# Amos-Chen98/neo-planner

Measured on NVIDIA B200. Metric: optimized trajectories/sec to convergence, higher is better.
Workload: dtype f64

## Files before the change

### neo_planner_b200/csrc/lbfgsb_tile.cuh

```cuda
#pragma once
#include "minco_tile.cuh"
#include "x87_nrm2.h"

namespace neo {

#ifdef NEO_OPT_TICKS
#define OT_BEGIN long long ot_last = clock64()
#define OT(i) do { const long long ot_now = clock64(); if (T.tl == 0) { atomicAdd((unsigned long long *)&g_opt_ticks[i], (unsigned long long)(ot_now - ot_last)); atomicAdd((unsigned long long *)&g_opt_ticks[32 + (i)], 1ull); } ot_last = clock64(); } while (0)
#else
#define OT_BEGIN do { } while (0)
#define OT(i) do { } while (0)
#endif

__device__ __forceinline__ double xmul(double a, double b) { return __dmul_rn(a, b); }
__device__ __forceinline__ double xadd(double a, double b) { return __dadd_rn(a, b); }
__device__ __forceinline__ double xsub(double a, double b) { return __dsub_rn(a, b); }
__device__ __noinline__ double xdiv(double a, double b) { return __ddiv_rn(a, b); }
__device__ __noinline__ double xsqrt(double a) { return __dsqrt_rn(a); }
__device__ __noinline__ double nrm2_x87(int n, const double *v) { return x87_nrm2(n, v); }
__device__ __forceinline__ double xrcp(double a) { return __drcp_rn(a); }
__device__ __forceinline__ double xfma(double a, double b, double c) { return __fma_rn(a, b, c); }
__device__ __forceinline__ double xdiv_r(double a, double b, double rb)
{
    const double q = __dmul_rn(a, rb);
// ... 377 lines not shown
#pragma unroll 1
    for (int i = m2 - 1; i >= 0; i--) {
        const double *ui = wn + wn_col(i);
        if (T.tl == 0) wv[i] = xdiv_r(wv[i], ui[i], rd[i]);
        T.sync();
        const double t = -wv[i];
#pragma unroll 1
        for (int k = T.tl; k < i; k += TL) wv[k] = xfma(t, ui[k], wv[k]);
        T.sync();
    }
    OT(10);
    if (T.tl < n) {
#pragma unroll 1
        for (int jy = 0; jy < col; jy++) {
            const int sj = lb_slot(L, jy);
            d = xadd(xadd(d, xdiv_r(xmul(m.wy[sj * n + T.tl], wv[jy]), theta, rtheta)), xmul(m.ws[sj * n + T.tl], wv[col + jy]));
        }
        d = xmul(d, rtheta);
    }
    T.sync();
    OT(11);
    return d;
}

template <int TL>
__device__ __forceinline__ void ls_load(const Tile<TL> &T, const double *p, Dcsrch &S)
{
    S.finit = p[0]; S.ginit = p[1]; S.gtest = p[2]; S.width = p[3]; S.width1 = p[4]; S.stx = p[5]; S.fx = p[6]; S.gx = p[7];
    S.sty = p[8]; S.fy = p[9]; S.gy = p[10]; S.stmin = p[11]; S.stmax = p[12];
    const int flags = (int)p[13];
    S.brackt = (flags & 1) != 0; S.stage = flags >> 1;
}
template <int TL>
__device__ __forceinline__ void ls_store(const Tile<TL> &T, double *p, const Dcsrch &S)
{
    T.sync();
    if (T.tl == 0) {
        p[0] = S.finit; p[1] = S.ginit; p[2] = S.gtest; p[3] = S.width; p[4] = S.width1; p[5] = S.stx; p[6] = S.fx; p[7] = S.gx;
        p[8] = S.sty; p[9] = S.fy; p[10] = S.gy; p[11] = S.stmin; p[12] = S.stmax;
        p[13] = (double)((S.brackt ? 1 : 0) | (S.stage << 1));
    }
    T.sync();
}

constexpr int ST_CANCELLED = 7;
constexpr int ST_RUNNING = -1;

struct OptState {
    double x, g, d, t, r, z, xlast;
    double f, stp, gd;
    LbMem L;
    int nit, nfev, ifun, status;
    bool first;
};

__device__ __forceinline__ void opt_begin(OptState &o, double x0l)
{
    o.x = x0l; o.g = 0.0; o.d = 0.0; o.t = 0.0; o.r = 0.0; o.z = 0.0; o.xlast = 0.0;
    o.f = 0.0; o.stp = 0.0; o.gd = 0.0;
    o.L.col = 0; o.L.head = 0; o.L.iupdat = 0; o.L.theta = 1.0;
    o.nit = 0; o.nfev = 0; o.ifun = 0; o.status = ST_RUNNING; o.first = true;
}

template <int TL>
__device__ __forceinline__ bool opt_same_point(const Tile<TL> &T, const OptState &o, int n)
{
    return !o.first && T.all(T.tl >= n || o.x == o.xlast);
}

template <int TL, int NC>
__device__ __forceinline__ double opt_gd(const Tile<TL> &T, const TileMem &m, int n, double g, double d)
{
    T.sync();
    if (T.tl < n) { m.gv[T.tl] = g; m.dv[T.tl] = d; }
    T.sync();
    return blas_ddot_n<NC>(m.gv, m.dv, n);
}

template <int TL, int NC>
__device__ __forceinline__ void opt_advance(const Tile<TL> &T, const TileMem &m, int n, OptState &o,
                                            const unsigned *cancel_word, unsigned cancel_mask)
{
    const bool mine = T.tl < n;
    const double pgtol = 1e-4, ftol = 1e-4, epsmch = 2.220446049250313e-16;
    const double tol = (ftol / epsmch) * epsmch;
    const int maxls = 20, maxiter = 15000, maxfun = 15000;
    bool new_dir;
    OT_BEGIN;
    if (o.first) {
        o.first = false;
        if (T.dmax(mine ? fabs(o.g) : 0.0) <= pgtol) { o.status = 1; return; }
        new_dir = true;
    } else {
        o.gd = opt_gd<TL, NC>(T, m, n, o.g, o.d);
        Dcsrch ls;
        ls_load(T, m.ls, ls);
        const int ls_task = dcsrch_step(ls, o.stp, o.f, o.gd);
        if (ls_task == 0) ls_store(T, m.ls, ls);
        OT(0);
        if (ls_task == 0) new_dir = false;
        else {
            o.nit++;
            if (cancel_mask) {
                unsigned w = 0;
                if (T.tl == 0) w = *reinterpret_cast<const volatile unsigned *>(cancel_word);
                if (T.shfl(w, 0) & cancel_mask) { o.status = ST_CANCELLED; return; }
            }
            if (T.dmax(mine ? fabs(o.g) : 0.0) <= pgtol) { o.status = 1; return; }
            const double fold = m.ls[14], gdold = m.ls[15];
            if (xsub(fold, o.f) <= xmul(tol, max3(fabs(fold), fabs(o.f), 1.0))) { o.status = 0; return; }
            if (o.nit >= maxiter || o.nfev > maxfun) { o.status = 3; return; }
            const double y = xsub(o.g, o.r);
            T.sync();
            if (mine) m.dv[T.tl] = y;
            T.sync();
            OT(12);
            const double nr = nrm2_x87(n, m.dv);
            const double rr = xmul(nr, nr);
            OT(1);
            double dr, ddum, s;
            if (o.stp == 1.0) { dr = xsub(o.gd, gdold); ddum = -gdold; s = o.d; }
            else { dr = xmul(xsub(o.gd, gdold), o.stp); s = xmul(o.d, o.stp); ddum = xmul(-gdold, o.stp); }
            if (!(dr <= xmul(epsmch, ddum))) lb_update<TL, NC>(T, m, n, o.L, s, y, rr, dr);
            new_dir = true;
        }
    }
    for (;;) {
        if (new_dir) {
            OT(15);
            if (o.L.col > 0 && !lb_factor(T, m, o.L)) { o.L.col = 0; o.L.head = 0; o.L.iupdat = 0; o.L.theta = 1.0; }
            if (o.L.col == 0) o.z = xsub(o.x, o.g);
            else o.z = xadd(o.x, lb_step<TL, NC>(T, m, n, o.L, o.g));
            o.d = mine ? xsub(o.z, o.x) : 0.0;
            T.sync();
            if (mine) m.dv[T.tl] = o.d;
            T.sync();
            OT(13);
            const double dnorm = nrm2_x87(n, m.dv);
            OT(1);
            o.stp = (o.nit == 0) ? fmin(xdiv(1.0, dnorm), LS_STPMAX) : 1.0;
            o.t = o.x; o.r = o.g;
            o.gd = opt_gd<TL, NC>(T, m, n, o.g, o.d);
            T.sync();
            if (T.tl == 0) { m.ls[14] = o.f; m.ls[15] = o.gd; }
            o.ifun = 0;
            if (o.gd >= 0.0) o.ifun = maxls + 1;
            else { Dcsrch ls; dcsrch_start(ls, o.stp, o.f, o.gd); ls_store(T, m.ls, ls); }
            OT(14);
        }
        o.ifun++;
        if (o.ifun - 1 < maxls) break;
        T.sync();
        o.x = o.t; o.g = o.r; o.f = m.ls[14];
        if (o.L.col == 0) { o.status = 2; return; }
        o.L.col = 0; o.L.head = 0; o.L.iupdat = 0; o.L.theta = 1.0;
        new_dir = true;
    }
    o.x = (o.stp == 1.0) ? o.z : xadd(xmul(o.stp, o.d), o.t);
}

}
```

### neo_planner_b200/csrc/neoopt.cu

```cuda
#include <cuda_runtime.h>
#include <math.h>
#include <stdio.h>
#include <stdlib.h>
#include <string.h>

#include <algorithm>
#include <atomic>
#include <chrono>
#include <condition_variable>
#include <functional>
#include <mutex>
#include <thread>
#include <string>
#include <vector>

#include "../../include/neoopt.h"
#include "astar_warp.cuh"
#include "lbfgsb_tile.cuh"
#include "map_kernels.cuh"
#include "minco_tile.cuh"

using namespace neo;

constexpr int WARPS_PER_CTA = 4;
#ifndef NEO_GROUPED_MIN_PROBLEMS
#define NEO_GROUPED_MIN_PROBLEMS 2048
#endif
#ifndef NEO_TILE_MIN_PROBLEMS
#define NEO_TILE_MIN_PROBLEMS 12288
#endif
#ifndef NEO_HOST_THREADS
#define NEO_HOST_THREADS 8
#endif

struct OptArgs {
    int B, M, max_attempts;
    const double *x0;
    const int32_t *x0_status;
    const double *head, *tail;
    const int32_t *map_ids;
    const double *retry_q;
    const double *retry_tau;
    int retry_status;
    const MapView *maps;
    unsigned int *counter;
    double *t_x;
    double *t_costs;
    int32_t *t_info;
    long long *t_work;
    unsigned int *p_state;
    double *x, *ts, *coeffs, *costs;
    int32_t *status, *ok, *attempt, *nit, *runs, *nfev;
    long long *work;
    int trace_cap;
    int bus_q;
    double *tr_x, *tr_f, *tr_g, *tr_costs;
    int32_t *tr_status, *tr_len;
};

__device__ __forceinline__ bool resolved(unsigned st, int A)
{
    const unsigned done = st & 0xffu, okm = (st >> 8) & 0xffu;
    if (okm) { const unsigned lower = (1u << (__ffs(okm) - 1)) - 1u; return (done & lower) == lower; }
    return done == (1u << A) - 1u;
}

#ifdef NEO_ROUND_TRACE
__device__ long long g_round_trace[12 * 2048 * 4];
#endif
template <int MODE, int MC, int TL, int MINB, int WPC = WARPS_PER_CTA>
__global__ void __launch_bounds__(WPC * 32, MINB) k_optimize(const DevParams P, const OptArgs a)
{
    extern __shared__ double smem[];
    const int lane = threadIdx.x & 31, warp = threadIdx.x >> 5;
    const Tile<TL> T(lane);
    constexpr int TPW = 32 / TL;
    const int M = MC > 0 ? MC : a.M, n = 3 * M - 2, nq = 2 * (M - 1), N = 6 * M, A = a.max_attempts;
    constexpr bool ONE_BLOCK = MODE == SAMPLE_BY_PIECE_STAGED;
    const TileMem m = carve(smem + (size_t)(warp * TPW + lane / TL) * tile_mem_doubles(M, TL, ONE_BLOCK), M, TL, ONE_BLOCK);
    const unsigned total = (unsigned)A * (unsigned)a.B;
    const bool mine = T.tl < n;
    OptState o;
    opt_begin(o, 0.0);
    bool running = false, retired = false;
    unsigned tid = 0, lower_ok = 0;
    int at = 0;
    size_t b = 0;
    int map_id = 0;
    unsigned long long t_start = 0;
    __shared__ unsigned s_arrivals;
    constexpr unsigned BUS_DRAIN = 0x80000000u;
    bool drained = false;
    if constexpr (WPC > WARPS_PER_CTA) {
        if (threadIdx.x == 0) s_arrivals = 0;
        __syncthreads();
    }
#ifdef NEO_ROUND_TRACE
    int rt_round = 0;
#endif
    for (;;) {
#ifdef NEO_ROUND_TRACE
        if (blockIdx.x == 0 && lane == 0 && rt_round < 2048) g_round_trace[(warp * 2048 + rt_round) * 4 + 0] = clock64();
#endif
        if constexpr (WPC > WARPS_PER_CTA) {
            __syncwarp();
            if (!drained) {
                unsigned k = 0;
                if (lane == 0) k = atomicAdd(&s_arrivals, 1u);
                k = __shfl_sync(FULL, k, 0);
                if (k & BUS_DRAIN) drained = true;
                else asm volatile("bar.sync %0, %1;" ::"r"(1 + (int)((k / (unsigned)a.bus_q) & 7u)), "r"(a.bus_q * 32) : "memory");
            }
        }
#ifdef NEO_ROUND_TRACE
        if (blockIdx.x == 0 && lane == 0 && rt_round < 2048) g_round_trace[(warp * 2048 + rt_round) * 4 + 1] = clock64();
        const int rt_now = rt_round++;
#endif
// ... 100 lines not shown
            }
            if (accepted) bits |= 1u << (8 + at);
            __threadfence();
        }
        T.sync();
        unsigned old = 0;
        if (T.tl == 0) old = atomicOr(a.p_state + b, bits);
        old = T.shfl(old, 0);
        const unsigned now = old | bits;
        if (!resolved(now, A) || resolved(old, A)) continue;

        __threadfence();
        const unsigned okm = (now >> 8) & 0xffu;
        const int last = okm ? __ffs(okm) - 1 : A - 1;
        int nit = 0, runs = 0, nfev = 0, src = -1, status = 0;
        long long ns = 0, nv = 0, nc = 0, nanos = 0;
        for (int k = 0; k <= last; k++) {
            const size_t t = (size_t)k * a.B + b;
            const int st = __ldcg(a.t_info + t * 4 + 0);
            status = st;
            nfev += __ldcg(a.t_info + t * 4 + 2);
            ns += __ldcg(a.t_work + t * 4 + 0); nv += __ldcg(a.t_work + t * 4 + 1); nc += __ldcg(a.t_work + t * 4 + 2);
            nanos += __ldcg(a.t_work + t * 4 + 3);
            if (__ldcg(a.t_info + t * 4 + 3)) { runs++; nit += __ldcg(a.t_info + t * 4 + 1); src = k; }
        }
        if (src >= 0) {
            const size_t t = (size_t)src * a.B + b;
            const double xf = mine ? __ldcg(a.t_x + t * n + T.tl) : 0.0;
            begin_problem(T, m, M, a.head + b * 6, a.tail + b * 6);
            double e_unused;
            times_from_tau(T, P, m, M, xf, e_unused);
            load_nodes(T, m, M, xf);
            solve_nodes(T, m, M);
            hermite_coeffs(T, m, M);
            if (mine) a.x[b * n + T.tl] = xf;
            if (T.tl < M) a.ts[b * M + T.tl] = m.ts[T.tl];
            for (int i = T.tl; i < 2 * N; i += TL) a.coeffs[b * 2 * N + i] = m.c[i];
            if (T.tl < 4) a.costs[b * 4 + T.tl] = __ldcg(a.t_costs + t * 4 + T.tl);
        } else {
            if (mine) a.x[b * n + T.tl] = 0.0;
            if (T.tl < M) a.ts[b * M + T.tl] = 0.0;
            for (int i = T.tl; i < 2 * N; i += TL) a.coeffs[b * 2 * N + i] = 0.0;
            if (T.tl < 4) a.costs[b * 4 + T.tl] = 0.0;
        }
        if (T.tl == 0) {
            a.status[b] = status; a.ok[b] = okm ? 1 : 0; a.attempt[b] = last; a.nit[b] = nit; a.runs[b] = runs;
            a.nfev[b] = nfev;
            if (a.work) { a.work[b * 4] = ns; a.work[b * 4 + 1] = nv; a.work[b * 4 + 2] = nc; a.work[b * 4 + 3] = nanos; }
        }
        T.sync();
    }
}

struct EvalArgs {
    int B, M;
    const double *x, *head, *tail;
    const int32_t *map_ids;
    const MapView *maps;
    double *costs, *grad, *coeffs, *ts;
    int32_t *status;
};

template <int MODE, int MC, int TL>
__global__ void __launch_bounds__(WARPS_PER_CTA * 32, 3) k_eval(const DevParams P, const EvalArgs a)
{
    extern __shared__ double smem[];
    const int lane = threadIdx.x & 31, warp = threadIdx.x >> 5;
    const Tile<TL> T(lane);
    constexpr int TPW = 32 / TL, TPC = WARPS_PER_CTA * TPW;
    const int M = MC > 0 ? MC : a.M, n = 3 * M - 2, N = 6 * M;
    const int tile = warp * TPW + lane / TL;
    constexpr bool ONE_BLOCK = MODE == SAMPLE_BY_PIECE_STAGED;
    const TileMem m = carve(smem + (size_t)tile * eval_mem_doubles(M, TL, ONE_BLOCK), M, TL, ONE_BLOCK, true);
    for (size_t b = (size_t)blockIdx.x * TPC + tile; b < (size_t)a.B; b += (size_t)gridDim.x * TPC) {
        begin_problem(T, m, M, a.head + b * 6, a.tail + b * 6);
        const MapView map = a.maps[a.map_ids ? a.map_ids[b] : 0];
        const double xl = T.tl < n ? a.x[b * n + T.tl] : 0.0;
        EvalOut ev;
        eval_fg<MODE, TL, true>(T, P, map, m, M, xl, true, ev);
        if (T.tl < n) a.grad[b * n + T.tl] = ev.status ? 0.0 : ev.g;
        if (T.tl < 4) a.costs[b * 4 + T.tl] = ev.costs[T.tl];
        if (T.tl == 0) a.status[b] = ev.status;
        if (a.coeffs) for (int i = T.tl; i < 2 * N; i += TL) a.coeffs[b * 2 * N + i] = ev.status == NEO_ST_OVERFLOW ? 0.0 : m.c[i];
        if (a.ts && T.tl < M) a.ts[b * M + T.tl] = m.ts[T.tl];
        T.sync();
    }
}

__global__ void __launch_bounds__(WARPS_PER_CTA * 32) k_coeffs(int B, int M, const double *q, const double *ts,
                                                               const double *head, const double *tail, double *coeffs)
{
    extern __shared__ double smem[];
    const int lane = threadIdx.x & 31, warp = threadIdx.x >> 5;
    const Tile<32> T(lane);
    const int nq = 2 * (M - 1), N = 6 * M;
    const TileMem m = carve(smem + (size_t)warp * tile_mem_doubles(M), M);
    for (size_t b = (size_t)blockIdx.x * WARPS_PER_CTA + warp; b < (size_t)B; b += (size_t)gridDim.x * WARPS_PER_CTA) {
        begin_problem(T, m, M, head + b * 6, tail + b * 6);
        if (lane < M) {
            const double Tt = ts[b * M + lane];
            m.ts[lane] = Tt;
            const double a = 1.0 / Tt, a2 = a * a;
            double *it = m.iT + 5 * lane;
            it[0] = a; it[1] = a2; it[2] = a2 * a; it[3] = a2 * a2; it[4] = a2 * a2 * a;
        }
        __syncwarp();
// ... 117 lines not shown
            }
        }
    }
    void loop()
    {
        unsigned long long seen = 0;
        for (;;) {
            {
                std::unique_lock<std::mutex> g(mu_);
                wake_.wait(g, [&] { return stop_ || generation_ != seen; });
                if (stop_) return;
                seen = generation_;
            }
            work();
        }
    }
    std::vector<std::thread> workers_;
    std::mutex mu_;
    std::condition_variable wake_, done_;
    const std::function<void(size_t, size_t)> *fn_ = nullptr;
    size_t count_ = 0, per_ = 0, parts_ = 0, next_ = 0, pending_ = 0;
    unsigned long long generation_ = 0;
    bool stop_ = false;
};

struct DevBuf {
    void *p = nullptr;
    size_t cap = 0;
};

struct neo_handle {
    int device = 0;
    cudaStream_t stream = nullptr;
    cudaEvent_t ev0 = nullptr, ev1 = nullptr;
    neo_config cfg;
    std::vector<MapSlot> slots;
    std::vector<MapView> views;
    MapView *d_maps = nullptr;
    unsigned int *d_counter = nullptr;
    std::vector<DevBuf> bufs;
    DevBuf pinned;
    DevBuf astar;
    size_t astar_cap = 0;
    int astar_warps = 0;
    size_t astar_laid_icap = 0;
    int astar_icap = 0;
    std::string err;
    std::mutex mu;
    float last_ms = 0.f;
    long long launches = 0;
    HostPool pool;
    bool host_timing = false;
    int grouped = -1, group_warps = 0;
    int tile = 0;
    int sm_count = 0, cc_major = 0, cc_minor = 0;
    char name[128] = {0};
};

static std::string g_create_err;

#define CK(call)                                                                                          \
    do {                                                                                                  \
        cudaError_t e_ = (call);                                                                          \
        if (e_ != cudaSuccess) {                                                                          \
            h->err = std::string(#call) + ": " + cudaGetErrorString(e_);                                  \
            return NEO_ERR_CUDA;                                                                          \
        }                                                                                                 \
    } while (0)

static int fail(neo_handle *h, const char *msg)
{
    h->err = msg;
    return NEO_ERR_INVALID;
}

static DevParams dev_params(const neo_config &c)
{
    DevParams P;
    P.v_max2 = c.v_max * c.v_max;
    P.T_min = c.T_min; P.T_max = c.T_max; P.safe_dis = c.safe_dis; P.dt = c.delta_t;
    P.w0 = c.weights[0]; P.w1 = c.weights[1]; P.w2 = c.weights[2]; P.w3 = c.weights[3];
    P.collision_cost_tol = c.collision_cost_tol;
    return P;
}

static int dev_buf(neo_handle *h, size_t i, size_t bytes, void **out)
{
    if (h->bufs.size() <= i) h->bufs.resize(i + 1);
    DevBuf &b = h->bufs[i];
    if (b.cap < bytes) {
        if (b.p) CK(cudaFree(b.p));
        b.p = nullptr; b.cap = 0;
        size_t cap = bytes + bytes / 4 + 256;
        CK(cudaMalloc(&b.p, cap));
        b.cap = cap;
    }
    *out = b.p;
    return NEO_OK;
}

static int pin_buf(neo_handle *h, size_t bytes, void **out)
{
    DevBuf &b = h->pinned;
    if (b.cap < bytes) {
        if (b.p) CK(cudaFreeHost(b.p));
        b.p = nullptr; b.cap = 0;
        const size_t cap = bytes + bytes / 4 + 256;
        CK(cudaHostAlloc(&b.p, cap, cudaHostAllocMapped));
        b.cap = cap;
    }
    *out = b.p;
    return NEO_OK;
}

static int cfg_check(const neo_config *c)
{
    return c && c->delta_t > 0.0 && c->T_max > c->T_min;
}

extern "C" int neo_create(const neo_config *cfg, int device, int max_maps, neo_handle **out)
{
    if (!out || !cfg_check(cfg) || max_maps < 1) { g_create_err = "neo_create: invalid argument"; return NEO_ERR_INVALID; }
    int ndev = 0;
    cudaError_t e = cudaGetDeviceCount(&ndev);
    if (e != cudaSuccess || ndev == 0 || device < 0 || device >= ndev) {
        g_create_err = std::string("neo_create: no usable CUDA device (") + cudaGetErrorString(e) +
                       "); libneoopt has no CPU fallback";
        return NEO_ERR_NO_DEVICE;
    }
    cudaDeviceProp prop;
    cudaGetDeviceProperties(&prop, device);
    if (prop.major < 10) {
        g_create_err = "neo_create: device is not sm_100 (Blackwell); this library ships sm_100a code only";
        return NEO_ERR_NO_DEVICE;
    }
    neo_handle *h = new neo_handle();
    h->device = device; h->cfg = *cfg; h->slots.resize(max_maps); h->views.resize(max_maps);
    h->host_timing = getenv("NEO_HOST_TIMING") != nullptr;
    if (const char *e = getenv("NEO_ASTAR_ICAP")) h->astar_icap = atoi(e);
    if (const char *e = getenv("NEO_GROUPED")) h->grouped = atoi(e) ? 1 : 0;
    if (const char *e = getenv("NEO_GROUP_WARPS")) h->group_warps = atoi(e);
    if (const char *e = getenv("NEO_TILE")) { const int t = atoi(e); h->tile = (t == 8 || t == 16 || t == 32) ? t : 0; }
    h->sm_count = prop.multiProcessorCount; h->cc_major = prop.major; h->cc_minor = prop.minor;
    snprintf(h->name, sizeof(h->name), "%s", prop.name);
    bool good = cudaSetDevice(device) == cudaSuccess &&
                cudaStreamCreateWithFlags(&h->stream, cudaStreamNonBlocking) == cudaSuccess &&
                cudaEventCreate(&h->ev0) == cudaSuccess && cudaEventCreate(&h->ev1) == cudaSuccess &&
                cudaMalloc(&h->d_maps, sizeof(MapView) * max_maps) == cudaSuccess &&
                cudaMemset(h->d_maps, 0, sizeof(MapView) * max_maps) == cudaSuccess &&
                cudaMalloc(&h->d_counter, sizeof(unsigned int) * 64) == cudaSuccess;
    if (!good) {
        g_create_err = std::string("neo_create: ") + cudaGetErrorString(cudaGetLastError());
        delete h;
        return NEO_ERR_CUDA;
    }
    *out = h;
    return NEO_OK;
}

extern "C" int neo_destroy(neo_handle *h)
{
    if (!h) return NEO_ERR_INVALID;
    cudaSetDevice(h->device);
    cudaStreamSynchronize(h->stream);
    for (auto &s : h->slots) { if (s.cells) cudaFree(s.cells); if (s.occ) cudaFree(s.occ); if (s.blocked) cudaFree(s.blocked); }
    for (auto &b : h->bufs) if (b.p) cudaFree(b.p);
    if (h->pinned.p) cudaFreeHost(h->pinned.p);
    if (h->astar.p) cudaFree(h->astar.p);
    cudaFree(h->d_maps); cudaFree(h->d_counter);
    cudaEventDestroy(h->ev0); cudaEventDestroy(h->ev1);
    cudaStreamDestroy(h->stream);
    delete h;
    return NEO_OK;
}

extern "C" int neo_set_config(neo_handle *h, const neo_config *cfg)
{
    if (!h) return NEO_ERR_INVALID;
    std::lock_guard<std::mutex> g(h->mu);
    if (!cfg_check(cfg)) return fail(h, "neo_set_config: invalid config");
    h->cfg = *cfg;
    return NEO_OK;
}

extern "C" const char *neo_last_error(neo_handle *h) { return h ? h->err.c_str() : g_create_err.c_str(); }

extern "C" int neo_device_info(neo_handle *h, int *sm_count, int *cc_major, int *cc_minor, char *name, int name_len)
{
    if (!h) return NEO_ERR_INVALID;
    if (sm_count) *sm_count = h->sm_count;
    if (cc_major) *cc_major = h->cc_major;
    if (cc_minor) *cc_minor = h->cc_minor;
    if (name && name_len > 0) snprintf(name, name_len, "%s", h->name);
    return NEO_OK;
}

// ... 228 lines not shown
}

static int check_problem(neo_handle *h, int B, int M)
{
    if (B < 0) return fail(h, "B must be >= 0");
    if (M < 2 || M > NEO_MAX_PIECES) return fail(h, "M must be in [2, NEO_MAX_PIECES]");
    if (!h->slots[0].cells) {
        bool any = false;
        for (auto &s : h->slots) any = any || s.cells;
        if (!any) return fail(h, "no map uploaded (neo_set_map_esdf / neo_set_map_occupancy)");
    }
    return NEO_OK;
}

static int check_map_ids(neo_handle *h, int B, const int32_t *map_ids, const char *who)
{
    if (!map_ids) {
        if (!h->slots[0].cells) { h->err = std::string(who) + ": map_ids is NULL and slot 0 holds no map"; return NEO_ERR_INVALID; }
        return NEO_OK;
    }
    for (int i = 0; i < B; i++)
        if (map_ids[i] < 0 || map_ids[i] >= (int)h->slots.size() || !h->slots[map_ids[i]].cells) {
            h->err = std::string(who) + ": map id " + std::to_string(map_ids[i]) + " (problem " + std::to_string(i) + ") refers to an empty slot";
            return NEO_ERR_INVALID;
        }
    return NEO_OK;
}

static size_t smem_bytes(int M, int TL = 32, bool one_block = false, int wpc = WARPS_PER_CTA)
{
    return sizeof(double) * (size_t)tile_mem_doubles(M, TL, one_block) * wpc * (32 / TL);
}

template <typename K>
static int prep_kernel(neo_handle *h, K kernel, size_t smem, int *ctas_per_sm, int wpc = WARPS_PER_CTA)
{
    CK(cudaFuncSetAttribute(kernel, cudaFuncAttributeMaxDynamicSharedMemorySize, (int)smem));
    int occ = 0;
    CK(cudaOccupancyMaxActiveBlocksPerMultiprocessor(&occ, kernel, wpc * 32, smem));
    if (occ < 1) return fail(h, "kernel does not fit on an SM");
    *ctas_per_sm = occ;
    return NEO_OK;
}

static int tile_lanes(const neo_handle *h, int B, int M)
{
    if (M > 4) return 32;
    const int small = M <= 3 ? 8 : 16;
    if (h->tile) return h->tile == 32 ? 32 : small;
    return B >= NEO_TILE_MIN_PROBLEMS ? small : 32;
}

typedef void (*OptKernel)(const DevParams, const OptArgs);
template <int MODE, int MC, int TL, int MINB>
static OptKernel pick_optimize(bool grouped, int *wpc)
{
    if (grouped) { *wpc = 4 * MINB; return k_optimize<MODE, MC, TL, 1, 4 * MINB>; }
    return k_optimize<MODE, MC, TL, MINB, WARPS_PER_CTA>;
}

static int launch_optimize(neo_handle *h, OptArgs a, cudaStream_t st)
{
    int occ;
    void (*kern)(const DevParams, const OptArgs) = nullptr;
    const int TL = tile_lanes(h, a.B, a.M);
    const bool staged = TL < 32;
    bool grouped = TL < 32 || a.B >= NEO_GROUPED_MIN_PROBLEMS;
    if (h->grouped >= 0) grouped = h->grouped != 0;
    int wpc = WARPS_PER_CTA;
#define NEO_PICK(MODE, MC, TLV, MINB) pick_optimize<MODE, MC, TLV, MINB>(grouped, &wpc)
#define NEO_KW(MODE, MC) NEO_PICK(MODE, MC, 32, 3)
    switch (a.M) {
#ifndef NEO_FAST_BUILD
        case 2: kern = TL == 8 ? NEO_PICK(SAMPLE_BY_PIECE_STAGED, 2, 8, 3) : NEO_KW(SAMPLE_BY_PIECE, 2); break;
        case 4: kern = TL == 16 ? NEO_PICK(SAMPLE_BY_PIECE_STAGED, 4, 16, 3) : NEO_KW(SAMPLE_BY_PIECE, 4); break;
        case 5: kern = NEO_KW(SAMPLE_ALL_PIECES, 5); break;
        case 6: kern = NEO_KW(SAMPLE_ALL_PIECES, 6); break;
        case 7: kern = NEO_KW(SAMPLE_ALL_PIECES, 7); break;
        case 8: kern = NEO_KW(SAMPLE_ALL_PIECES, 8); break;
        case 9: kern = NEO_KW(SAMPLE_ALL_PIECES, 9); break;
        case 10: kern = NEO_KW(SAMPLE_ALL_PIECES, 10); break;
#endif
        case 3: kern = TL == 8 ? NEO_PICK(SAMPLE_BY_PIECE_STAGED, 3, 8, 3) : NEO_KW(SAMPLE_BY_PIECE, 3); break;
        default: return fail(h, "M must be in [2, NEO_MAX_PIECES]");
    }
#undef NEO_KW
#undef NEO_PICK
    a.bus_q = h->group_warps > 0 ? h->group_warps : 3 * wpc / 4;
    if (a.bus_q > wpc) a.bus_q = wpc;
    const size_t smem = smem_bytes(a.M, TL, staged, wpc);
    int rc = prep_kernel(h, kern, smem, &occ, wpc);
    if (rc) return rc;
    const size_t tasks = (size_t)a.B * a.max_attempts, n = 3 * a.M - 2;
    const size_t per_cta = (size_t)wpc * (32 / TL);
    const size_t need = (tasks + per_cta - 1) / per_cta;
    const int grid = (int)(need < (size_t)occ * h->sm_count ? need : (size_t)occ * h->sm_count);
    char *base;
    const size_t o_x = 0, o_c = o_x + sizeof(double) * tasks * n, o_w = o_c + sizeof(double) * tasks * 4,
                 o_i = o_w + sizeof(long long) * tasks * 4, o_p = o_i + sizeof(int32_t) * tasks * 4,
                 total = o_p + sizeof(unsigned) * a.B;
    if ((rc = dev_buf(h, 6, total, (void **)&base))) return rc;
    a.t_x = (double *)(base + o_x); a.t_costs = (double *)(base + o_c); a.t_work = (long long *)(base + o_w);
    a.t_info = (int32_t *)(base + o_i); a.p_state = (unsigned *)(base + o_p);
    a.maps = h->d_maps;
    a.counter = h->d_counter;
    CK(cudaMemsetAsync(h->d_counter, 0, sizeof(unsigned int), st));
    CK(cudaMemsetAsync(a.p_state, 0, sizeof(unsigned) * a.B, st));
    kern<<<grid, wpc * 32, smem, st>>>(dev_params(h->cfg), a);
    h->launches++;
    CK(cudaGetLastError());
    return NEO_OK;
}

static int launch_eval(neo_handle *h, EvalArgs a, cudaStream_t st)
{
    int occ;
    void (*kern)(const DevParams, const EvalArgs) = nullptr;
    const int TL = tile_lanes(h, a.B, a.M);
    switch (a.M) {
#ifndef NEO_FAST_BUILD
        case 2: kern = TL == 8 ? k_eval<SAMPLE_BY_PIECE_STAGED, 2, 8> : k_eval<SAMPLE_BY_PIECE, 2, 32>; break;
        case 4: kern = TL == 16 ? k_eval<SAMPLE_BY_PIECE_STAGED, 4, 16> : k_eval<SAMPLE_BY_PIECE, 4, 32>; break;
        case 5: kern = k_eval<SAMPLE_ALL_PIECES, 5, 32>; break;
        case 6: kern = k_eval<SAMPLE_ALL_PIECES, 6, 32>; break;
        case 7: kern = k_eval<SAMPLE_ALL_PIECES, 7, 32>; break;
        case 8: kern = k_eval<SAMPLE_ALL_PIECES, 8, 32>; break;
        case 9: kern = k_eval<SAMPLE_ALL_PIECES, 9, 32>; break;
        case 10: kern = k_eval<SAMPLE_ALL_PIECES, 10, 32>; break;
#endif
        case 3: kern = TL == 8 ? k_eval<SAMPLE_BY_PIECE_STAGED, 3, 8> : k_eval<SAMPLE_BY_PIECE, 3, 32>; break;
        default: return fail(h, "M must be in [2, NEO_MAX_PIECES]");
    }
    const size_t smem = sizeof(double) * (size_t)eval_mem_doubles(a.M, TL, TL < 32) * WARPS_PER_CTA * (32 / TL);
    int rc = prep_kernel(h, kern, smem, &occ);
    if (rc) return rc;
    const int per_cta = WARPS_PER_CTA * (32 / TL);
    const int need = (a.B + per_cta - 1) / per_cta;
    const int grid = need < occ * h->sm_count ? need : occ * h->sm_count;
    a.maps = h->d_maps;
    kern<<<grid, WARPS_PER_CTA * 32, smem, st>>>(dev_params(h->cfg), a);
    h->launches++;
    CK(cudaGetLastError());
    return NEO_OK;
}

struct Carver {
    char *base;
    size_t off = 0;
    template <typename T>
    T *take(size_t count)
    {
        off = (off + 255) & ~(size_t)255;
        T *p = base ? (T *)(base + off) : nullptr;
        off += sizeof(T) * count;
        return p;
    }
// ... 652 lines not shown
```

Measured before the change: 2.434 million.

## Add slot-pool optimizer kernel that batches tiles by phase across shared-memory slots

Splits the L-BFGS-B step into an after-evaluation phase and a direction phase. It then adds a persistent pool kernel in which many problem slots live in shared memory, with per-slot state spilled to global records. Each warp claims several ready slots that are in the same phase, grouping direction-phase slots by L-BFGS column count, so the sub-warp tiles within a warp follow the same code path instead of diverging. This becomes the default for small-tile (TL<32) launches. The cost is global round-trips for the state on every phase and scheduling overhead on shared atomics.

```diff
diff --git a/neo_planner_b200/csrc/lbfgsb_tile.cuh b/neo_planner_b200/csrc/lbfgsb_tile.cuh
--- a/neo_planner_b200/csrc/lbfgsb_tile.cuh
+++ b/neo_planner_b200/csrc/lbfgsb_tile.cuh
@@ -453,6 +453,7 @@
     LbMem L;
     int nit, nfev, ifun, status;
     bool first;
+    bool upd;
 };
 
 __device__ __forceinline__ void opt_begin(OptState &o, double x0l)
@@ -460,7 +461,7 @@
     o.x = x0l; o.g = 0.0; o.d = 0.0; o.t = 0.0; o.r = 0.0; o.z = 0.0; o.xlast = 0.0;
     o.f = 0.0; o.stp = 0.0; o.gd = 0.0;
     o.L.col = 0; o.L.head = 0; o.L.iupdat = 0; o.L.theta = 1.0;
-    o.nit = 0; o.nfev = 0; o.ifun = 0; o.status = ST_RUNNING; o.first = true;
+    o.nit = 0; o.nfev = 0; o.ifun = 0; o.status = ST_RUNNING; o.first = true; o.upd = false;
 }
 
 template <int TL>
@@ -476,88 +477,113 @@
     if (T.tl < n) { m.gv[T.tl] = g; m.dv[T.tl] = d; }
     T.sync();
     return blas_ddot_n<NC>(m.gv, m.dv, n);
+}
+
+constexpr double OPT_PGTOL = 1e-4, OPT_EPSMCH = 2.220446049250313e-16;
+constexpr int OPT_MAXLS = 20;
+
+__device__ __forceinline__ void opt_trial(OptState &o) { o.x = (o.stp == 1.0) ? o.z : xadd(xmul(o.stp, o.d), o.t); }
+
+template <int TL, int NC>
+__device__ __forceinline__ bool opt_after_eval(const Tile<TL> &T, const TileMem &m, int n, OptState &o,
+                                               const unsigned *cancel_word, unsigned cancel_mask)
+{
+    const bool mine = T.tl < n;
+    const double ftol = 1e-4;
+    const double tol = (ftol / OPT_EPSMCH) * OPT_EPSMCH;
+    const int maxiter = 15000, maxfun = 15000;
+    OT_BEGIN;
+    if (o.first) {
+        o.first = false;
+        if (T.dmax(mine ? fabs(o.g) : 0.0) <= OPT_PGTOL) { o.status = 1; return false; }
+        return true;
+    }
+    o.gd = opt_gd<TL, NC>(T, m, n, o.g, o.d);
+    Dcsrch ls;
+    ls_load(T, m.ls, ls);
+    const int ls_task = dcsrch_step(ls, o.stp, o.f, o.gd);
+    if (ls_task == 0) ls_store(T, m.ls, ls);
+    OT(0);
+    if (ls_task == 0) {
+        o.ifun++;
+        if (o.ifun - 1 < OPT_MAXLS) { opt_trial(o); return false; }
+        T.sync();
+        o.x = o.t; o.g = o.r; o.f = m.ls[14];
+        if (o.L.col == 0) { o.status = 2; return false; }
+        o.L.col = 0; o.L.head = 0; o.L.iupdat = 0; o.L.theta = 1.0;
+        return true;
+    }
+    o.nit++;
+    if (cancel_mask) {
+        unsigned w = 0;
+        if (T.tl == 0) w = *reinterpret_cast<const volatile unsigned *>(cancel_word);
+        if (T.shfl(w, 0) & cancel_mask) { o.status = ST_CANCELLED; return false; }
+    }
+    if (T.dmax(mine ? fabs(o.g) : 0.0) <= OPT_PGTOL) { o.status = 1; return false; }
+    const double fold = m.ls[14];
+    if (xsub(fold, o.f) <= xmul(tol, max3(fabs(fold), fabs(o.f), 1.0))) { o.status = 0; return false; }
+    if (o.nit >= maxiter || o.nfev > maxfun) { o.status = 3; return false; }
+    o.upd = true;
+    return true;
+}
+
+template <int TL, int NC>
+__device__ __forceinline__ void opt_direction(const Tile<TL> &T, const TileMem &m, int n, OptState &o)
+{
+    const bool mine = T.tl < n;
+    OT_BEGIN;
+    if (o.upd) {
+        o.upd = false;
+        const double gdold = m.ls[15];
+        const double y = xsub(o.g, o.r);
+        T.sync();
+        if (mine) m.dv[T.tl] = y;
+        T.sync();
+        OT(12);
+        const double nr = nrm2_x87(n, m.dv);
+        const double rr = xmul(nr, nr);
+        OT(1);
+        double dr, ddum, s;
+        if (o.stp == 1.0) { dr = xsub(o.gd, gdold); ddum = -gdold; s = o.d; }
+        else { dr = xmul(xsub(o.gd, gdold), o.stp); s = xmul(o.d, o.stp); ddum = xmul(-gdold, o.stp); }
+        if (!(dr <= xmul(OPT_EPSMCH, ddum))) lb_update<TL, NC>(T, m, n, o.L, s, y, rr, dr);
+    }
+    for (;;) {
+        OT(15);
+        if (o.L.col > 0 && !lb_factor(T, m, o.L)) { o.L.col = 0; o.L.head = 0; o.L.iupdat = 0; o.L.theta = 1.0; }
+        if (o.L.col == 0) o.z = xsub(o.x, o.g);
+        else o.z = xadd(o.x, lb_step<TL, NC>(T, m, n, o.L, o.g));
+        o.d = mine ? xsub(o.z, o.x) : 0.0;
+        T.sync();
+        if (mine) m.dv[T.tl] = o.d;
+        T.sync();
+        OT(13);
+        const double dnorm = nrm2_x87(n, m.dv);
+        OT(1);
+        o.stp = (o.nit == 0) ? fmin(xdiv(1.0, dnorm), LS_STPMAX) : 1.0;
+        o.t = o.x; o.r = o.g;
+        o.gd = opt_gd<TL, NC>(T, m, n, o.g, o.d);
+        T.sync();
+        if (T.tl == 0) { m.ls[14] = o.f; m.ls[15] = o.gd; }
+        o.ifun = 0;
+        if (o.gd >= 0.0) o.ifun = OPT_MAXLS + 1;
+        else { Dcsrch ls; dcsrch_start(ls, o.stp, o.f, o.gd); ls_store(T, m.ls, ls); }
+        OT(14);
+        o.ifun++;
+        if (o.ifun - 1 < OPT_MAXLS) break;
+        T.sync();
+        o.x = o.t; o.g = o.r; o.f = m.ls[14];
+        if (o.L.col == 0) { o.status = 2; return; }
+        o.L.col = 0; o.L.head = 0; o.L.iupdat = 0; o.L.theta = 1.0;
+    }
+    opt_trial(o);
 }
 
 template <int TL, int NC>
 __device__ __forceinline__ void opt_advance(const Tile<TL> &T, const TileMem &m, int n, OptState &o,
                                             const unsigned *cancel_word, unsigned cancel_mask)
 {
-    const bool mine = T.tl < n;
-    const double pgtol = 1e-4, ftol = 1e-4, epsmch = 2.220446049250313e-16;
-    const double tol = (ftol / epsmch) * epsmch;
-    const int maxls = 20, maxiter = 15000, maxfun = 15000;
-    bool new_dir;
-    OT_BEGIN;
-    if (o.first) {
-        o.first = false;
-        if (T.dmax(mine ? fabs(o.g) : 0.0) <= pgtol) { o.status = 1; return; }
-        new_dir = true;
-    } else {
-        o.gd = opt_gd<TL, NC>(T, m, n, o.g, o.d);
-        Dcsrch ls;
-        ls_load(T, m.ls, ls);
-        const int ls_task = dcsrch_step(ls, o.stp, o.f, o.gd);
-        if (ls_task == 0) ls_store(T, m.ls, ls);
-        OT(0);
-        if (ls_task == 0) new_dir = false;
-        else {
-            o.nit++;
-            if (cancel_mask) {
-                unsigned w = 0;
-                if (T.tl == 0) w = *reinterpret_cast<const volatile unsigned *>(cancel_word);
-                if (T.shfl(w, 0) & cancel_mask) { o.status = ST_CANCELLED; return; }
-            }
-            if (T.dmax(mine ? fabs(o.g) : 0.0) <= pgtol) { o.status = 1; return; }
-            const double fold = m.ls[14], gdold = m.ls[15];
-            if (xsub(fold, o.f) <= xmul(tol, max3(fabs(fold), fabs(o.f), 1.0))) { o.status = 0; return; }
-            if (o.nit >= maxiter || o.nfev > maxfun) { o.status = 3; return; }
-            const double y = xsub(o.g, o.r);
-            T.sync();
-            if (mine) m.dv[T.tl] = y;
-            T.sync();
-            OT(12);
-            const double nr = nrm2_x87(n, m.dv);
-            const double rr = xmul(nr, nr);
-            OT(1);
-            double dr, ddum, s;
-            if (o.stp == 1.0) { dr = xsub(o.gd, gdold); ddum = -gdold; s = o.d; }
-            else { dr = xmul(xsub(o.gd, gdold), o.stp); s = xmul(o.d, o.stp); ddum = xmul(-gdold, o.stp); }
-            if (!(dr <= xmul(epsmch, ddum))) lb_update<TL, NC>(T, m, n, o.L, s, y, rr, dr);
-            new_dir = true;
-        }
-    }
-    for (;;) {
-        if (new_dir) {
-            OT(15);
-            if (o.L.col > 0 && !lb_factor(T, m, o.L)) { o.L.col = 0; o.L.head = 0; o.L.iupdat = 0; o.L.theta = 1.0; }
-            if (o.L.col == 0) o.z = xsub(o.x, o.g);
-            else o.z = xadd(o.x, lb_step<TL, NC>(T, m, n, o.L, o.g));
-            o.d = mine ? xsub(o.z, o.x) : 0.0;
-            T.sync();
-            if (mine) m.dv[T.tl] = o.d;
-            T.sync();
-            OT(13);
-            const double dnorm = nrm2_x87(n, m.dv);
-            OT(1);
-            o.stp = (o.nit == 0) ? fmin(xdiv(1.0, dnorm), LS_STPMAX) : 1.0;
-            o.t = o.x; o.r = o.g;
-            o.gd = opt_gd<TL, NC>(T, m, n, o.g, o.d);
-            T.sync();
-            if (T.tl == 0) { m.ls[14] = o.f; m.ls[15] = o.gd; }
-            o.ifun = 0;
-            if (o.gd >= 0.0) o.ifun = maxls + 1;
-            else { Dcsrch ls; dcsrch_start(ls, o.stp, o.f, o.gd); ls_store(T, m.ls, ls); }
-            OT(14);
-        }
-        o.ifun++;
-        if (o.ifun - 1 < maxls) break;
-        T.sync();
-        o.x = o.t; o.g = o.r; o.f = m.ls[14];
-        if (o.L.col == 0) { o.status = 2; return; }
-        o.L.col = 0; o.L.head = 0; o.L.iupdat = 0; o.L.theta = 1.0;
-        new_dir = true;
-    }
-    o.x = (o.stp == 1.0) ? o.z : xadd(xmul(o.stp, o.d), o.t);
-}
-
-}
+    if (opt_after_eval<TL, NC>(T, m, n, o, cancel_word, cancel_mask)) opt_direction<TL, NC>(T, m, n, o);
+}
+
+}
diff --git a/neo_planner_b200/csrc/neoopt.cu b/neo_planner_b200/csrc/neoopt.cu
--- a/neo_planner_b200/csrc/neoopt.cu
+++ b/neo_planner_b200/csrc/neoopt.cu
@@ -54,6 +54,8 @@
     long long *work;
     int trace_cap;
     int bus_q;
+    int pool_slots;
+    double *pool;
     double *tr_x, *tr_f, *tr_g, *tr_costs;
     int32_t *tr_status, *tr_len;
 };
@@ -63,6 +65,151 @@
     const unsigned done = st & 0xffu, okm = (st >> 8) & 0xffu;
     if (okm) { const unsigned lower = (1u << (__ffs(okm) - 1)) - 1u; return (done & lower) == lower; }
     return done == (1u << A) - 1u;
+}
+
+struct Task {
+    unsigned tid, lower_ok;
+    int at, map_id;
+    size_t b;
+    unsigned long long t_start;
+};
+
+template <int TL>
+__device__ __forceinline__ bool task_claim(const Tile<TL> &T, const OptArgs &a, const TileMem &m, int M, Task &k, OptState &o,
+                                           bool &run, bool &report)
+{
+    const int n = 3 * M - 2, nq = 2 * (M - 1), A = a.max_attempts;
+    const bool mine = T.tl < n;
+    unsigned t0 = 0;
+    if (T.tl == 0) t0 = atomicAdd(a.counter, 1u);
+    k.tid = T.shfl(t0, 0);
+    if (k.tid >= (unsigned)A * (unsigned)a.B) return false;
+    k.at = (int)(k.tid / (unsigned)a.B);
+    k.b = k.tid - (unsigned)k.at * (unsigned)a.B;
+    k.lower_ok = ((1u << k.at) - 1u) << 8;
+    unsigned seen = 0;
+    if (T.tl == 0) seen = *reinterpret_cast<volatile unsigned *>(a.p_state + k.b);
+    seen = T.shfl(seen, 0);
+    run = false; report = false;
+    if (!(seen & k.lower_ok)) {
+        asm volatile("mov.u64 %0, %%globaltimer;" : "=l"(k.t_start));
+        begin_problem(T, m, M, a.head + k.b * 6, a.tail + k.b * 6);
+        k.map_id = a.map_ids ? a.map_ids[k.b] : 0;
+        double x0l = 0.0;
+        int st0 = 0;
+        if (k.at == 0) {
+            if (mine) x0l = a.x0[k.b * n + T.tl];
+            st0 = a.x0_status ? a.x0_status[k.b] : 0;
+        } else {
+            if (T.tl < nq) x0l = a.retry_q[(k.b * (A - 1) + (k.at - 1)) * nq + T.tl];
+            else if (mine) x0l = a.retry_tau[T.tl - nq];
+            st0 = a.retry_status;
+        }
+        opt_begin(o, x0l);
+        if (T.tl < 7) m.oc[T.tl] = 0.0;
+        T.sync();
+        report = true;
+        if (st0) { o.status = st0; o.x = 0.0; }
+        else run = true;
+    }
+    return true;
+}
+
+template <int MODE, int TL>
+__device__ __forceinline__ bool eval_site(const Tile<TL> &T, const DevParams &P, const OptArgs &a, const TileMem &m, int M,
+                                          const Task &k, OptState &o)
+{
+    const int n = 3 * M - 2;
+    const bool mine = T.tl < n;
+    if (opt_same_point(T, o, n)) return true;
+    EvalOut ev;
+    OT_BEGIN;
+    eval_fg<MODE, TL>(T, P, a.maps[k.map_id], m, M, o.x, true, ev);
+    OT(16);
+    if (T.tl == 0) { m.oc[4] += (double)ev.ns; m.oc[5] += (double)ev.nv; m.oc[6] += (double)ev.nc; }
+    if (a.tr_x && o.nfev < a.trace_cap) {
+        const size_t t = (size_t)k.tid * a.trace_cap + o.nfev;
+        if (mine) { a.tr_x[t * n + T.tl] = o.x; a.tr_g[t * n + T.tl] = ev.status ? 0.0 : ev.g; }
+        if (T.tl < 4) a.tr_costs[t * 4 + T.tl] = ev.costs[T.tl];
+        if (T.tl == 0) { a.tr_f[t] = ev.f; a.tr_status[t] = ev.status; a.tr_len[k.tid] = o.nfev + 1; }
+    }
+    if (ev.status) { o.status = ev.status; return false; }
+    o.f = ev.f; o.g = mine ? ev.g : 0.0; o.nfev++; o.xlast = o.x;
+    if (T.tl < 4) m.oc[T.tl] = ev.costs[T.tl];
+    return true;
+}
+
+template <int TL>
+__device__ __forceinline__ void task_end(const Tile<TL> &T, const DevParams &P, const OptArgs &a, const TileMem &m, int M,
+                                         const Task &k, const OptState &o, bool report)
+{
+    const int n = 3 * M - 2, N = 6 * M, A = a.max_attempts;
+    const bool mine = T.tl < n;
+    const size_t b = k.b;
+    unsigned bits = 1u << k.at;
+    if (report && o.status != ST_CANCELLED) {
+        const bool completed = o.status < NEO_ST_OVERFLOW;
+        T.sync();
+        const bool accepted = completed && !(m.oc[3] * P.w3 > P.collision_cost_tol);
+        if (mine) a.t_x[(size_t)k.tid * n + T.tl] = o.x;
+        if (T.tl < 4) a.t_costs[(size_t)k.tid * 4 + T.tl] = m.oc[T.tl];
+        if (T.tl == 0) {
+            a.t_info[(size_t)k.tid * 4 + 0] = o.status; a.t_info[(size_t)k.tid * 4 + 1] = o.nit;
+            a.t_info[(size_t)k.tid * 4 + 2] = o.nfev; a.t_info[(size_t)k.tid * 4 + 3] = completed ? 1 : 0;
+            unsigned long long t_end;
+            asm volatile("mov.u64 %0, %%globaltimer;" : "=l"(t_end));
+            a.t_work[(size_t)k.tid * 4 + 0] = (long long)m.oc[4]; a.t_work[(size_t)k.tid * 4 + 1] = (long long)m.oc[5];
+            a.t_work[(size_t)k.tid * 4 + 2] = (long long)m.oc[6]; a.t_work[(size_t)k.tid * 4 + 3] = (long long)(t_end - k.t_start);
+        }
+        if (accepted) bits |= 1u << (8 + k.at);
+        __threadfence();
+    }
+    T.sync();
+    unsigned old = 0;
+    if (T.tl == 0) old = atomicOr(a.p_state + b, bits);
+    old = T.shfl(old, 0);
+    const unsigned now = old | bits;
+    if (!resolved(now, A) || resolved(old, A)) return;
+
+    __threadfence();
+    const unsigned okm = (now >> 8) & 0xffu;
+    const int last = okm ? __ffs(okm) - 1 : A - 1;
+    int nit = 0, runs = 0, nfev = 0, src = -1, status = 0;
+    long long ns = 0, nv = 0, nc = 0, nanos = 0;
+    for (int q = 0; q <= last; q++) {
+        const size_t t = (size_t)q * a.B + b;
+        const int st = __ldcg(a.t_info + t * 4 + 0);
+        status = st;
+        nfev += __ldcg(a.t_info + t * 4 + 2);
+        ns += __ldcg(a.t_work + t * 4 + 0); nv += __ldcg(a.t_work + t * 4 + 1); nc += __ldcg(a.t_work + t * 4 + 2);
+        nanos += __ldcg(a.t_work + t * 4 + 3);
+        if (__ldcg(a.t_info + t * 4 + 3)) { runs++; nit += __ldcg(a.t_info + t * 4 + 1); src = q; }
+    }
+    if (src >= 0) {
+        const size_t t = (size_t)src * a.B + b;
+        const double xf = mine ? __ldcg(a.t_x + t * n + T.tl) : 0.0;
+        begin_problem(T, m, M, a.head + b * 6, a.tail + b * 6);
+        double e_unused;
+        times_from_tau(T, P, m, M, xf, e_unused);
+        load_nodes(T, m, M, xf);
+        solve_nodes(T, m, M);
+        hermite_coeffs(T, m, M);
+        if (mine) a.x[b * n + T.tl] = xf;
+        if (T.tl < M) a.ts[b * M + T.tl] = m.ts[T.tl];
+        for (int i = T.tl; i < 2 * N; i += TL) a.coeffs[b * 2 * N + i] = m.c[i];
+        if (T.tl < 4) a.costs[b * 4 + T.tl] = __ldcg(a.t_costs + t * 4 + T.tl);
+    } else {
+        if (mine) a.x[b * n + T.tl] = 0.0;
+        if (T.tl < M) a.ts[b * M + T.tl] = 0.0;
+        for (int i = T.tl; i < 2 * N; i += TL) a.coeffs[b * 2 * N + i] = 0.0;
+        if (T.tl < 4) a.costs[b * 4 + T.tl] = 0.0;
+    }
+    if (T.tl == 0) {
+        a.status[b] = status; a.ok[b] = okm ? 1 : 0; a.attempt[b] = last; a.nit[b] = nit; a.runs[b] = runs;
+        a.nfev[b] = nfev;
+        if (a.work) { a.work[b * 4] = ns; a.work[b * 4 + 1] = nv; a.work[b * 4 + 2] = nc; a.work[b * 4 + 3] = nanos; }
+    }
+    T.sync();
 }
 
 #ifdef NEO_ROUND_TRACE
@@ -269,6 +416,176 @@
     }
 }
 
+constexpr int POOL_MAX_SLOTS = 64;
+#ifndef NEO_POOL_PATIENCE
+#define NEO_POOL_PATIENCE 0
+#endif
+constexpr int POOL_EVAL = 0, POOL_DIR = 1, POOL_EMPTY = 2;
+
+struct PoolScalars {
+    double f, stp, gd, theta;
+    unsigned long long t_start;
+    int col, head, iupdat, nit, nfev, ifun, status, flags;
+    unsigned tid;
+    int map_id;
+};
+__host__ __device__ constexpr int pool_rec_doubles(int TL) { return 7 * TL + (int)(sizeof(PoolScalars) / sizeof(double)); }
+
+template <int TL>
+__device__ __forceinline__ void pool_store(const Tile<TL> &T, double *r, const OptState &o, const Task &k)
+{
+    const int l = T.tl;
+    __stcg(r + 0 * TL + l, o.x); __stcg(r + 1 * TL + l, o.g); __stcg(r + 2 * TL + l, o.d); __stcg(r + 3 * TL + l, o.t);
+    __stcg(r + 4 * TL + l, o.r); __stcg(r + 5 * TL + l, o.z); __stcg(r + 6 * TL + l, o.xlast);
+    if (l == 0) {
+        PoolScalars *p = reinterpret_cast<PoolScalars *>(r + 7 * TL);
+        __stcg(&p->f, o.f); __stcg(&p->stp, o.stp); __stcg(&p->gd, o.gd); __stcg(&p->theta, o.L.theta);
+        __stcg(&p->t_start, k.t_start);
+        __stcg(&p->col, o.L.col); __stcg(&p->head, o.L.head); __stcg(&p->iupdat, o.L.iupdat);
+        __stcg(&p->nit, o.nit); __stcg(&p->nfev, o.nfev); __stcg(&p->ifun, o.ifun); __stcg(&p->status, o.status);
+        __stcg(&p->flags, (o.first ? 1 : 0) | (o.upd ? 2 : 0));
+        __stcg(&p->tid, k.tid); __stcg(&p->map_id, k.map_id);
+    }
+}
+
+template <int TL>
+__device__ __forceinline__ void pool_load(const Tile<TL> &T, const double *r, const OptArgs &a, OptState &o, Task &k)
+{
+    const int l = T.tl;
+    o.x = __ldcg(r + 0 * TL + l); o.g = __ldcg(r + 1 * TL + l); o.d = __ldcg(r + 2 * TL + l); o.t = __ldcg(r + 3 * TL + l);
+    o.r = __ldcg(r + 4 * TL + l); o.z = __ldcg(r + 5 * TL + l); o.xlast = __ldcg(r + 6 * TL + l);
+    const PoolScalars *p = reinterpret_cast<const PoolScalars *>(r + 7 * TL);
+    o.f = __ldcg(&p->f); o.stp = __ldcg(&p->stp); o.gd = __ldcg(&p->gd); o.L.theta = __ldcg(&p->theta);
+    k.t_start = __ldcg(&p->t_start);
+    o.L.col = __ldcg(&p->col); o.L.head = __ldcg(&p->head); o.L.iupdat = __ldcg(&p->iupdat);
+    o.nit = __ldcg(&p->nit); o.nfev = __ldcg(&p->nfev); o.ifun = __ldcg(&p->ifun); o.status = __ldcg(&p->status);
+    const int flags = __ldcg(&p->flags);
+    o.first = (flags & 1) != 0; o.upd = (flags & 2) != 0;
+    k.tid = __ldcg(&p->tid); k.map_id = __ldcg(&p->map_id);
+    k.at = (int)(k.tid / (unsigned)a.B);
+    k.b = k.tid - (unsigned)k.at * (unsigned)a.B;
+    k.lower_ok = ((1u << k.at) - 1u) << 8;
+}
+
+template <int TL>
+__device__ __forceinline__ int pool_refill(const Tile<TL> &T, const DevParams &P, const OptArgs &a, const TileMem &m, int M,
+                                           Task &k, OptState &o)
+{
+    for (;;) {
+        bool run, report;
+        if (!task_claim(T, a, m, M, k, o, run, report)) return POOL_EMPTY;
+        if (run) return POOL_EVAL;
+        task_end(T, P, a, m, M, k, o, report);
+    }
+}
+
+template <int TL>
+__device__ __forceinline__ void pool_release(const Tile<TL> &T, double *r, int s, int next, const OptState &o, const Task &k,
+                                             unsigned long long *ready, int *live, volatile unsigned char *col)
+{
+    if (next != POOL_EMPTY) pool_store(T, r, o, k);
+    __threadfence_block();
+    T.sync();
+    if (T.tl == 0) {
+        if (next == POOL_EMPTY) atomicSub(live, 1);
+        else { col[s] = (unsigned char)o.L.col; atomicOr(ready + next, 1ull << s); }
+    }
+}
+
+__device__ __forceinline__ unsigned long long lowest_bits(unsigned long long v, int k)
+{
+    unsigned long long r = 0;
+    for (int i = 0; i < k && v; i++) { const unsigned long long lo = v & (~v + 1ull); r |= lo; v ^= lo; }
+    return r;
+}
+
+template <int MODE, int MC, int TL, int WPC>
+__global__ void __launch_bounds__(WPC * 32, 1) k_optimize_pool(const DevParams P, const OptArgs a)
+{
+    extern __shared__ double smem[];
+    __shared__ unsigned long long s_ready[2];
+    __shared__ int s_live;
+    __shared__ unsigned char s_col[POOL_MAX_SLOTS];
+    const int lane = threadIdx.x & 31, warp = threadIdx.x >> 5;
+    const Tile<TL> T(lane);
+    constexpr int TPW = 32 / TL, NC = MC > 0 ? 3 * MC - 2 : 0;
+    constexpr bool ONE_BLOCK = MODE == SAMPLE_BY_PIECE_STAGED;
+    const int M = MC > 0 ? MC : a.M, n = 3 * M - 2, S = a.pool_slots;
+    const size_t slot_doubles = tile_mem_doubles(M, TL, ONE_BLOCK);
+    double *const recs = a.pool + (size_t)blockIdx.x * S * pool_rec_doubles(TL);
+    if (threadIdx.x == 0) { s_ready[POOL_EVAL] = 0; s_ready[POOL_DIR] = 0; s_live = S; }
+    __syncthreads();
+    for (int s = warp * TPW + lane / TL; s < S; s += WPC * TPW) {
+        const TileMem m = carve(smem + s * slot_doubles, M, TL, ONE_BLOCK);
+        OptState o;
+        Task k;
+        const int next = pool_refill(T, P, a, m, M, k, o);
+        pool_release(T, recs + s * pool_rec_doubles(TL), s, next, o, k, s_ready, &s_live, s_col);
+    }
+    int idle = 0;
+    for (;;) {
+        __syncwarp();
+        unsigned long long got = 0;
+        int pass = POOL_EVAL, quit = 0;
+        if (lane == 0) {
+            const unsigned long long ev = *reinterpret_cast<volatile unsigned long long *>(&s_ready[POOL_EVAL]);
+            const unsigned long long dr = *reinterpret_cast<volatile unsigned long long *>(&s_ready[POOL_DIR]);
+            const int ne = __popcll(ev), nd = __popcll(dr);
+            const bool full = nd >= TPW || ne >= TPW;
+            if ((ev | dr) && (full || idle >= NEO_POOL_PATIENCE)) {
+                pass = nd >= TPW ? POOL_DIR : (ne >= TPW ? POOL_EVAL : (nd >= ne ? POOL_DIR : POOL_EVAL));
+                const unsigned long long avail = pass == POOL_DIR ? dr : ev;
+                unsigned long long want = avail;
+                if (pass == POOL_DIR && TPW > 1) {
+                    const int c = s_col[__ffsll(avail) - 1];
+                    unsigned long long same = 0;
+                    for (unsigned long long v = avail; v; v &= v - 1) {
+                        const int s = __ffsll(v) - 1;
+                        if (s_col[s] == c) same |= 1ull << s;
+                    }
+                    want = lowest_bits(same, TPW);
+                    want |= lowest_bits(avail & ~want, TPW - __popcll(want));
+                } else want = lowest_bits(avail, TPW);
+                got = atomicAnd(&s_ready[pass], ~want) & want;
+            } else if (!(ev | dr)) quit = *reinterpret_cast<volatile int *>(&s_live) == 0;
+            idle = got ? 0 : idle + 1;
+#ifdef NEO_OPT_TICKS
+            if (got) { atomicAdd((unsigned long long *)&g_opt_ticks[26 + 2 * pass], 1ull); atomicAdd((unsigned long long *)&g_opt_ticks[27 + 2 * pass], (unsigned long long)__popcll(got)); }
+            else atomicAdd((unsigned long long *)&g_opt_ticks[30], 1ull);
+#endif
+        }
+        got = __shfl_sync(FULL, got, 0);
+        pass = __shfl_sync(FULL, pass, 0);
+        if (__shfl_sync(FULL, quit, 0)) break;
+        if (!got) { __nanosleep(256); continue; }
+        __threadfence_block();
+        unsigned long long g = got;
+        for (int i = 0; i < lane / TL; i++) g &= g - 1;
+        if (!g) continue;
+        const int s = __ffsll(g) - 1;
+        const TileMem m = carve(smem + s * slot_doubles, M, TL, ONE_BLOCK);
+        double *const r = recs + s * pool_rec_doubles(TL);
+        OptState o;
+        Task k;
+        pool_load(T, r, a, o, k);
+        bool ended;
+        int next = POOL_EVAL;
+        if (pass == POOL_EVAL) {
+            if (!eval_site<MODE>(T, P, a, m, M, k, o)) ended = true;
+            else if (opt_after_eval<TL, NC>(T, m, n, o, a.p_state + k.b, k.lower_ok)) { ended = false; next = POOL_DIR; }
+            else ended = o.status != ST_RUNNING;
+        } else {
+            opt_direction<TL, NC>(T, m, n, o);
+            ended = o.status != ST_RUNNING;
+        }
+        if (ended) {
+            task_end(T, P, a, m, M, k, o, true);
+            next = pool_refill(T, P, a, m, M, k, o);
+        }
+        pool_release(T, r, s, next, o, k, s_ready, &s_live, s_col);
+    }
+}
+
 struct EvalArgs {
     int B, M;
     const double *x, *head, *tail;
@@ -492,6 +809,8 @@
     HostPool pool;
     bool host_timing = false;
     int grouped = -1, group_warps = 0;
+    int slot_pool = -1;
+    int smem_optin = 0;
     int tile = 0;
     int sm_count = 0, cc_major = 0, cc_minor = 0;
     char name[128] = {0};
@@ -580,8 +899,10 @@
     if (const char *e = getenv("NEO_ASTAR_ICAP")) h->astar_icap = atoi(e);
     if (const char *e = getenv("NEO_GROUPED")) h->grouped = atoi(e) ? 1 : 0;
     if (const char *e = getenv("NEO_GROUP_WARPS")) h->group_warps = atoi(e);
+    if (const char *e = getenv("NEO_POOL")) h->slot_pool = atoi(e) ? 1 : 0;
     if (const char *e = getenv("NEO_TILE")) { const int t = atoi(e); h->tile = (t == 8 || t == 16 || t == 32) ? t : 0; }
     h->sm_count = prop.multiProcessorCount; h->cc_major = prop.major; h->cc_minor = prop.minor;
+    h->smem_optin = (int)prop.sharedMemPerBlockOptin;
     snprintf(h->name, sizeof(h->name), "%s", prop.name);
     bool good = cudaSetDevice(device) == cudaSuccess &&
                 cudaStreamCreateWithFlags(&h->stream, cudaStreamNonBlocking) == cudaSuccess &&
@@ -916,9 +1237,14 @@
 }
 
 typedef void (*OptKernel)(const DevParams, const OptArgs);
+#ifndef NEO_POOL_WARPS
+#define NEO_POOL_WARPS 12
+#endif
+constexpr int POOL_WARPS = NEO_POOL_WARPS;
 template <int MODE, int MC, int TL, int MINB>
-static OptKernel pick_optimize(bool grouped, int *wpc)
-{
+static OptKernel pick_optimize(bool pool, bool grouped, int *wpc)
+{
+    if (pool) { *wpc = POOL_WARPS; return k_optimize_pool<MODE, MC, TL, POOL_WARPS>; }
     if (grouped) { *wpc = 4 * MINB; return k_optimize<MODE, MC, TL, 1, 4 * MINB>; }
     return k_optimize<MODE, MC, TL, MINB, WARPS_PER_CTA>;
 }
@@ -931,8 +1257,10 @@
     const bool staged = TL < 32;
     bool grouped = TL < 32 || a.B >= NEO_GROUPED_MIN_PROBLEMS;
     if (h->grouped >= 0) grouped = h->grouped != 0;
+    bool pool = TL < 32;
+    if (h->slot_pool >= 0) pool = h->slot_pool != 0;
     int wpc = WARPS_PER_CTA;
-#define NEO_PICK(MODE, MC, TLV, MINB) pick_optimize<MODE, MC, TLV, MINB>(grouped, &wpc)
+#define NEO_PICK(MODE, MC, TLV, MINB) pick_optimize<MODE, MC, TLV, MINB>(pool, grouped, &wpc)
 #define NEO_KW(MODE, MC) NEO_PICK(MODE, MC, 32, 3)
     switch (a.M) {
 #ifndef NEO_FAST_BUILD
@@ -952,20 +1280,25 @@
 #undef NEO_PICK
     a.bus_q = h->group_warps > 0 ? h->group_warps : 3 * wpc / 4;
     if (a.bus_q > wpc) a.bus_q = wpc;
-    const size_t smem = smem_bytes(a.M, TL, staged, wpc);
+    const size_t slot_bytes = sizeof(double) * (size_t)tile_mem_doubles(a.M, TL, staged);
+    a.pool_slots = pool ? (int)std::min<size_t>(POOL_MAX_SLOTS, (size_t)(h->smem_optin - 1024) / slot_bytes) : 0;
+    if (pool && a.pool_slots < 1) return fail(h, "a pool slot does not fit in shared memory");
+    const size_t smem = pool ? slot_bytes * a.pool_slots : smem_bytes(a.M, TL, staged, wpc);
     int rc = prep_kernel(h, kern, smem, &occ, wpc);
     if (rc) return rc;
     const size_t tasks = (size_t)a.B * a.max_attempts, n = 3 * a.M - 2;
-    const size_t per_cta = (size_t)wpc * (32 / TL);
+    const size_t per_cta = pool ? (size_t)a.pool_slots : (size_t)wpc * (32 / TL);
     const size_t need = (tasks + per_cta - 1) / per_cta;
     const int grid = (int)(need < (size_t)occ * h->sm_count ? need : (size_t)occ * h->sm_count);
     char *base;
     const size_t o_x = 0, o_c = o_x + sizeof(double) * tasks * n, o_w = o_c + sizeof(double) * tasks * 4,
                  o_i = o_w + sizeof(long long) * tasks * 4, o_p = o_i + sizeof(int32_t) * tasks * 4,
-                 total = o_p + sizeof(unsigned) * a.B;
+                 o_r = (o_p + sizeof(unsigned) * a.B + 255) & ~(size_t)255,
+                 total = o_r + (pool ? sizeof(double) * (size_t)grid * a.pool_slots * pool_rec_doubles(TL) : 0);
     if ((rc = dev_buf(h, 6, total, (void **)&base))) return rc;
     a.t_x = (double *)(base + o_x); a.t_costs = (double *)(base + o_c); a.t_work = (long long *)(base + o_w);
     a.t_info = (int32_t *)(base + o_i); a.p_state = (unsigned *)(base + o_p);
+    a.pool = pool ? (double *)(base + o_r) : nullptr;
     a.maps = h->d_maps;
     a.counter = h->d_counter;
     CK(cudaMemsetAsync(h->d_counter, 0, sizeof(unsigned int), st));
```

After: 2.131 million, median of 6. 0.875x the previous value.
